# solislemuslab/BayesianNetworkRegression.jl

Measured on AMD Instinct MI355X. Metric: Gibbs iterations/sec (all chains), higher is better.
Workload: dtype f64; 1 GPU; synthetic n=500 V=100 (q=5050) R=7, 8 chains total, 8 per GPU; chains_total=8, chains_per_gpu=8, seed=20240501

## Files before the change

### bayesiannetworkregression.jl_amd/csrc/bnr_kernels.h

```cpp
#pragma once
#include "bnr_device.h"

#define BNR_RMAX 32
#define BNR_NB 32
#define BNR_GT 64


#define BNR_GLOBAL_PTR(member) d.member = (decltype(d.member))(__attribute__((address_space(1))) void *)(unsigned long long)(d.member)
__device__ __forceinline__ bnr_dev bnr_globalized(const bnr_dev *src)
{
    bnr_dev d = *src;
    BNR_GLOBAL_PTR(X); BNR_GLOBAL_PTR(X8); BNR_GLOBAL_PTR(XM); BNR_GLOBAL_PTR(Sdig); BNR_GLOBAL_PTR(y); BNR_GLOBAL_PTR(ek); BNR_GLOBAL_PTR(el); BNR_GLOBAL_PTR(trace); BNR_GLOBAL_PTR(plan);
    BNR_GLOBAL_PTR(pbase); BNR_GLOBAL_PTR(Wbuf); BNR_GLOBAL_PTR(sz); BNR_GLOBAL_PTR(PW); BNR_GLOBAL_PTR(PA); BNR_GLOBAL_PTR(PG);
    BNR_GLOBAL_PTR(Gpart); BNR_GLOBAL_PTR(E); BNR_GLOBAL_PTR(gmap); BNR_GLOBAL_PTR(a3); BNR_GLOBAL_PTR(xw); BNR_GLOBAL_PTR(a4);
    BNR_GLOBAL_PTR(res); BNR_GLOBAL_PTR(xg); BNR_GLOBAL_PTR(bw); BNR_GLOBAL_PTR(wv); BNR_GLOBAL_PTR(scal); BNR_GLOBAL_PTR(Minv);
    BNR_GLOBAL_PTR(Psum); BNR_GLOBAL_PTR(counters); BNR_GLOBAL_PTR(dbg); BNR_GLOBAL_PTR(stamp); BNR_GLOBAL_PTR(gprog); BNR_GLOBAL_PTR(gmapc); BNR_GLOBAL_PTR(dfctl);
    return d;
}
struct bnr_one {
    bnr_dev d;
    static constexpr bool whole = true, lone = true;
    __device__ __forceinline__ const bnr_dev &get() const { return d; }
    __device__ __forceinline__ const bnr_dev &get_x() const { return d; }
    __device__ __forceinline__ const bnr_dev &at(int) const { return d; }
// ... 423 lines not shown
            int f = wave_chol(sA, R, lane);
            if (f && lane == 0) { atomicAdd((unsigned long long *)&cd.counters[3], 1ull); atomicAdd((unsigned long long *)&cd.counters[6], 1ull); }
            const double lgm = (lane < R) ? 2.0 * log(sA[lane + R * lane]) : 0.0;
            double ldm = 0.0;
            for (int i = 0; i < R; ++i) ldm += bnr_readlane_u(lgm, i);
            wave_tri_inverse(sA, sT, R, lane);
            for (int idx = lane; idx < RR; idx += 64) {
                int a = idx % R, b = idx / R, k0 = a > b ? a : b;
                double sacc = 0.0;
                for (int k = k0; k < R; ++k) sacc += sT[k + R * a] * sT[k + R * b];
                cd.Minv[idx] = sacc;
            }
            if (lane == 0) cd.Minv[RR] = ldm;
        }
    }
    if (cap) atomicAdd((unsigned long long *)&cd.counters[2], 1ull);
}

template <class SRC>
__global__ __launch_bounds__(256) void k_xpass(const SRC chain_src, int s, int which, int nchains)
{
    extern __shared__ double sh[];
    const int gid = blockIdx.x;
    const int gx = gid & 7, gr = gid >> 3;
    const int bid = (gr / nchains) * 8 + gx;
    const bnr_dev &cd = chain_src.at(gr % nchains);
    if (bid >= cd.nblk_x) return;
    BNR_TL_IN(cd, TL_XPASS, bid == 0);
    double *sW = sh, *sZ = sh + cd.chunk_x, *sG = sh + 2 * cd.chunk_x;
    const bnr_plan_entry P = cd.plan[cd.pbase[0] + s];
    const double *row = cd.trace + (size_t)P.row * cd.rowlen;
    const double *prev = cd.trace + (size_t)P.prev * cd.rowlen;
    const int R = cd.R;
    const int e0 = bid * cd.chunk_x;
    const int ne = min(cd.chunk_x, cd.q - e0);
    const double *grow = (which & 8) ? prev : row;
    for (int t = threadIdx.x; t < cd.chunk_x; t += blockDim.x) {
        double w = 0.0, zz = 0.0, g = 0.0;
        int e = e0 + t;
        if (t < ne) {
            if (which & 1) { w = edge_W(row + cd.o_u, prev + cd.o_lam, R, cd.el[e], cd.ek[e]); cd.Wbuf[e] = w; }
            if (which & 2) { zz = sqrt(prev[cd.o_S + e]) * bnr_normal(cd.seed, P.it, SITE_G_Z1, (uint32_t)e, 0); cd.sz[e] = zz; }
            if (which & 4) g = grow[cd.o_gamma + e];
        }
        sW[t] = w; sZ[t] = zz; sG[t] = g;
    }
    __syncthreads();
    const size_t ld = cd.n_pad;
    for (int i = threadIdx.x; i < cd.n_pad; i += blockDim.x) {
        double aw = 0.0, aa = 0.0, ag = 0.0;
#define BNR_XPASS_BODY(XP)                                                                                          \
        if ((which & 7) == 3) {                                                                                     \
            _Pragma("unroll 4") for (int t = 0; t < ne; ++t) { double x = (double)(XP)[(size_t)t * ld]; aw = fma(x, sW[t], aw); aa = fma(x, sZ[t], aa); } \
        } else {                                                                                                    \
            for (int t = 0; t < ne; ++t) {                                                                          \
                double x = (double)(XP)[(size_t)t * ld];                                                            \
                aw = fma(x, sW[t], aw); aa = fma(x, sZ[t], aa); ag = fma(x, sG[t], ag);                             \
            }                                                                                                       \
        }
        if (cd.X8) { const unsigned char *xp = cd.X8 + (size_t)e0 * ld + i; BNR_XPASS_BODY(xp) }
        else { const double *xp = cd.X + (size_t)e0 * ld + i; BNR_XPASS_BODY(xp) }
        if (which & 1) cd.PW[(size_t)bid * ld + i] = aw;
        if (which & 2) cd.PA[(size_t)bid * ld + i] = aa;
        if (which & 4) cd.PG[(size_t)bid * ld + i] = ag;
    }
    BNR_TL_OUT(cd, TL_XPASS);
}

__global__ __launch_bounds__(256) void k_xpass_group(const bnr_many chain_src, int s, int nchains)
{
    extern __shared__ double sh[];
    const int wg = blockIdx.x;
    const bnr_dev &c0 = chain_src.at(0);
    const int rs = (c0.n_pad + 255) / 256, bid = wg / rs, slice = wg % rs, tid = threadIdx.x;
    const int chunk = c0.chunk_x, e0 = bid * chunk, ne = min(chunk, c0.q - e0), R = c0.R;
    const size_t ld = c0.n_pad;
    double *sW = sh, *sZ = sh + 8 * chunk;
    __shared__ double *s_pw[8], *s_pa[8];
    const int i = slice * 256 + tid;
    const bool live = i < c0.n_pad;
    const int ic = live ? i : 0;
    for (int cb = 0; cb < nchains; cb += 8) {
        const int nc = min(8, nchains - cb);
        __syncthreads();
        for (int it = tid; it < nc * chunk; it += 256) {
            const int c = it / chunk, t = it - c * chunk;
            const bnr_dev &cd = chain_src.at(cb + c);
            const bnr_plan_entry P = cd.plan[cd.pbase[0] + s];
            const double *row = cd.trace + (size_t)P.row * cd.rowlen, *prev = cd.trace + (size_t)P.prev * cd.rowlen;
            double w = 0.0, zz = 0.0;
            if (t < ne) {
                const int e = e0 + t;
                w = edge_W(row + cd.o_u, prev + cd.o_lam, R, cd.el[e], cd.ek[e]);
                zz = sqrt(prev[cd.o_S + e]) * bnr_normal(cd.seed, P.it, SITE_G_Z1, (uint32_t)e, 0);
                if (slice == 0) { cd.Wbuf[e] = w; cd.sz[e] = zz; }
            }
            sW[c * chunk + t] = w; sZ[c * chunk + t] = zz;
        }
        if (tid < nc) { const bnr_dev &cd = chain_src.at(cb + tid); s_pw[tid] = cd.PW; s_pa[tid] = cd.PA; }
        __syncthreads();
        double aw[8], aa[8];
#pragma unroll
        for (int c = 0; c < 8; ++c) { aw[c] = 0.0; aa[c] = 0.0; }
#define BNR_XG_BODY(XP)                                                                                   \
        for (int t0 = 0; t0 < ne; t0 += 16) {                                                             \
            double xv[16];                                                                                \
            _Pragma("unroll") for (int u = 0; u < 16; ++u) xv[u] = (double)(XP)[(size_t)(t0 + u < ne ? t0 + u : ne - 1) * ld]; \
            _Pragma("unroll") for (int u = 0; u < 16; ++u) {                                              \
                if (t0 + u < ne) {                                                                        \
                    _Pragma("unroll") for (int c = 0; c < 8; ++c)                                         \
                        if (c < nc) { aw[c] = fma(xv[u], sW[c * chunk + t0 + u], aw[c]); aa[c] = fma(xv[u], sZ[c * chunk + t0 + u], aa[c]); } \
                }                                                                                         \
            }                                                                                             \
        }
        if (c0.X8) { const unsigned char *xp = c0.X8 + (size_t)e0 * ld + ic; BNR_XG_BODY(xp) }
        else { const double *xp = c0.X + (size_t)e0 * ld + ic; BNR_XG_BODY(xp) }
#pragma unroll
        for (int c = 0; c < 8; ++c)
            if (c < nc && live) { s_pw[c][(size_t)bid * ld + i] = aw[c]; s_pa[c][(size_t)bid * ld + i] = aa[c]; }
    }
}

typedef int bnr_i4 __attribute__((ext_vector_type(4)));
typedef int bnr_i2 __attribute__((ext_vector_type(2)));
__device__ __forceinline__ __amdgpu_buffer_rsrc_t bnr_rsrc(const void *base)
{
    return __builtin_amdgcn_make_buffer_rsrc((void *)base, 0, 0x7FFFFFFF, 0x00020000);
}
__device__ __forceinline__ bnr_d2 bnr_bufload_d2(__amdgpu_buffer_rsrc_t r, unsigned voff, int soff)
{
    return __builtin_bit_cast(bnr_d2, __builtin_amdgcn_raw_buffer_load_b128(r, (int)voff, soff, 0));
}
__device__ __forceinline__ double bnr_bufload_f64(__amdgpu_buffer_rsrc_t r, unsigned voff, int soff)
{
    return __builtin_bit_cast(double, __builtin_amdgcn_raw_buffer_load_b64(r, (int)voff, soff, 0));
}
__device__ __forceinline__ void bnr_gram_count(const bnr_dev &cd, int tj)
{
    (void)cd; (void)tj;
}
#define BNR_GRAM_KB 16
#define BNR_GRAM_LOOKAHEAD 2
#define BNR_GRAM_PREFETCH_COLS 64
static_assert((BNR_GRAM_LOOKAHEAD + 1) * BNR_GRAM_KB <= BNR_GRAM_PREFETCH_COLS, "zero padding behind X and S must cover the Gram loops' prefetch distance (a half batch + two whole ones)");
__host__ __device__ inline long long bnr_gram_span_bytes(int n_pad, int kchunk, int kg)
{
    return ((long long)(kchunk / kg) + BNR_GRAM_PREFETCH_COLS + 16) * (long long)n_pad * 8;
}

__device__ __forceinline__ void bnr_gstore(double *p, double v) { *p = v; }
struct bnr_gram_geom { const double *X; int n_pad, q_pad, ksplit, q, ntile; };
__device__ __forceinline__ bnr_gram_geom bnr_geom_of(const bnr_dev &cd) { return bnr_gram_geom{cd.X, cd.n_pad, cd.q_pad, cd.ksplit, cd.q, cd.ntile}; }
template <int KG>
__device__ __forceinline__ void bnr_gram16_task(const bnr_gram_geom &cd, const double *Sp, double *Gpart, int t, int ti, int tj, int ks, double *sred)
{
    const int wave = threadIdx.x >> 6, lane = threadIdx.x & 63;
    const int kg = wave >> 2, wi = (wave >> 1) & 1, wj = wave & 1;
    const int kchunk = cd.q_pad / cd.ksplit;
    const int ksub = kchunk / KG;
    const int eb = ks * kchunk + kg * ksub;
    const int nfull = ksub / BNR_GRAM_KB;
    const bool half = (ksub % BNR_GRAM_KB) != 0;
    const size_t ld = cd.n_pad;
    const int li = lane & 15, lk = lane >> 4;
    const int tg = threadIdx.x & 255, c = tg >> 5, rp = tg & 31;
    const unsigned offI = 8u * ((unsigned)(ti * BNR_GT + 2 * rp) + (unsigned)c * (unsigned)ld), offJ = 8u * ((unsigned)(tj * BNR_GT + 2 * rp) + (unsigned)c * (unsigned)ld);
    const unsigned off8 = 8u * 8u * (unsigned)ld, offS = 8u * (unsigned)c;
    const double *xb = bnr_sgpr_global(cd.X + (size_t)eb * ld);
    const double *sb = bnr_sgpr_global(Sp + eb);
    const int PANEL = BNR_GRAM_KB * BNR_GT;
    double *stg = sred + (size_t)kg * (4 * PANEL);
    const int woff = c * BNR_GT + ((2 * rp) ^ ((c & 1) << 4));
    const int sw = (lk & 1) << 4;
    const int ra0 = (wj * 32 + li) ^ sw, ra1 = (wj * 32 + 16 + li) ^ sw, rb0 = (wi * 32 + li) ^ sw, rb1 = (wi * 32 + 16 + li) ^ sw;
    bnr_d4 c00 = {0, 0, 0, 0}, c01 = {0, 0, 0, 0}, c10 = {0, 0, 0, 0}, c11 = {0, 0, 0, 0};
    bnr_d2 ri0, ri1, rj0, rj1;
    double sv0, sv1;
    const __amdgpu_buffer_rsrc_t rX = bnr_rsrc(xb), rS = bnr_rsrc(sb);
    const int bstep = BNR_GRAM_KB * (int)ld * 8;
#define BNR_GRAM_LOAD(BIDX)                                                                               \
    do {                                                                                                  \
        const int so_ = (BIDX) * bstep;                                                                   \
        sv0 = bnr_bufload_f64(rS, offS, (BIDX) * (BNR_GRAM_KB * 8)); sv1 = bnr_bufload_f64(rS, offS + 64u, (BIDX) * (BNR_GRAM_KB * 8)); \
        ri0 = bnr_bufload_d2(rX, offI, so_); ri1 = bnr_bufload_d2(rX, offI + off8, so_);                  \
        rj0 = bnr_bufload_d2(rX, offJ, so_); rj1 = bnr_bufload_d2(rX, offJ + off8, so_);                  \
    } while (0)
#define BNR_GRAM_STORE(BUF)                                                                               \
    do {                                                                                                  \
        double *nx_ = stg + (size_t)(BUF) * (2 * PANEL);                                                  \
        *(bnr_d2 *)(nx_ + woff) = ri0 * sv0;                                                          \
        *(bnr_d2 *)(nx_ + 8 * BNR_GT + woff) = ri1 * sv1;                                             \
        *(bnr_d2 *)(nx_ + PANEL + woff) = rj0;                                                            \
        *(bnr_d2 *)(nx_ + PANEL + 8 * BNR_GT + woff) = rj1;                                               \
    } while (0)
#define BNR_GRAM_COMPUTE(BUF, K2A, K2B, DIAG)                                                                 \
    do {                                                                                                  \
        const double *bufI = stg + (size_t)(BUF) * (2 * PANEL), *bufJ = bufI + PANEL;                     \
        _Pragma("unroll") for (int k2 = (K2A); k2 < (K2B); ++k2) {                                        \
            const int kk = (4 * k2 + lk) * BNR_GT;                                                        \
            double a0 = bufJ[kk + ra0], a1 = bufJ[kk + ra1];                                              \
            double b0 = bufI[kk + rb0], b1 = bufI[kk + rb1];                                              \
            c00 = __builtin_amdgcn_mfma_f64_16x16x4f64(a0, b0, c00, 0, 0, 0);                             \
            c01 = __builtin_amdgcn_mfma_f64_16x16x4f64(a0, b1, c01, 0, 0, 0);                             \
            if (!(DIAG)) c10 = __builtin_amdgcn_mfma_f64_16x16x4f64(a1, b0, c10, 0, 0, 0);                \
            c11 = __builtin_amdgcn_mfma_f64_16x16x4f64(a1, b1, c11, 0, 0, 0);                             \
        }                                                                                                 \
    } while (0)
    BNR_GRAM_LOAD(0);
    BNR_GRAM_STORE(0);
    BNR_GRAM_LOAD(1);
    __syncthreads();
    if (ti == tj && wi == 0 && wj == 1) {
        int b = 0;
        for (; b + 1 < nfull; b += 2) {
            BNR_GRAM_STORE(1); BNR_GRAM_LOAD(b + 2); __syncthreads();
            BNR_GRAM_STORE(0); BNR_GRAM_LOAD(b + 3); __syncthreads();
        }
        if (b < nfull) { BNR_GRAM_STORE(1); BNR_GRAM_LOAD(b + 2); __syncthreads(); }
        if (half) __syncthreads();
    } else if (ti == tj && wi == wj) {
#define BNR_GRAM_BATCH_L(B, PAR, DIAG)                                                                    \
        do {                                                                                              \
            BNR_GRAM_COMPUTE(PAR, 0, 2, DIAG);                                                            \
            BNR_GRAM_STORE((PAR) ^ 1);                                                                    \
            BNR_GRAM_LOAD((B) + 2);                                                                       \
            BNR_GRAM_COMPUTE(PAR, 2, 4, DIAG);                                                            \
            __syncthreads();                                                                              \
        } while (0)
        int b = 0;
        for (; b + 1 < nfull; b += 2) { BNR_GRAM_BATCH_L(b, 0, true); BNR_GRAM_BATCH_L(b + 1, 1, true); }
        if (b < nfull) BNR_GRAM_BATCH_L(b, 0, true);
        if (half) { if (nfull & 1) BNR_GRAM_COMPUTE(1, 0, 2, true); else BNR_GRAM_COMPUTE(0, 0, 2, true); __syncthreads(); }
    } else {
    int b = 0;
    for (; b + 1 < nfull; b += 2) { BNR_GRAM_BATCH_L(b, 0, false); BNR_GRAM_BATCH_L(b + 1, 1, false); }
    if (b < nfull) BNR_GRAM_BATCH_L(b, 0, false);
    if (half) { if (nfull & 1) BNR_GRAM_COMPUTE(1, 0, 2, false); else BNR_GRAM_COMPUTE(0, 0, 2, false); __syncthreads(); }
    }
    double *mine = sred + (size_t)kg * (BNR_GT * BNR_GT);
    const int jb = wj * 32 + (lane >> 4), ib = wi * 32 + (lane & 15);
#pragma unroll
    for (int r = 0; r < 4; ++r) {
        mine[(jb + 4 * r) * BNR_GT + ib] = c00[r];
        mine[(jb + 4 * r) * BNR_GT + ib + 16] = c01[r];
        mine[(jb + 16 + 4 * r) * BNR_GT + ib] = c10[r];
        mine[(jb + 16 + 4 * r) * BNR_GT + ib + 16] = c11[r];
    }
    __syncthreads();
    double *out = Gpart + ((size_t)ks * (cd.ntile * (cd.ntile + 1) / 2) + t) * (BNR_GT * BNR_GT);
#pragma unroll
    for (int idx = threadIdx.x; idx < BNR_GT * BNR_GT; idx += KG * 256) {
        if (KG == 4) bnr_gstore(out + idx, (sred[idx] + sred[BNR_GT * BNR_GT + idx]) + (sred[2 * BNR_GT * BNR_GT + idx] + sred[3 * BNR_GT * BNR_GT + idx]));
        else bnr_gstore(out + idx, sred[idx] + sred[BNR_GT * BNR_GT + idx]);
    }
}
template <class SRC, int KG>
__global__ __launch_bounds__(KG * 256, 4 / KG) void k_gram(const SRC chain_src, int s, int nchains)
{
    const int gid = blockIdx.x, gx = gid & 7, gr = gid >> 3;
    const int gchain = gr % nchains, gslot = (gr / nchains) * 8 + gx;
    const bnr_dev &cd = chain_src.at(gchain);
    __shared__ double sred[KG * BNR_GT * BNR_GT];
    const bnr_plan_entry P = cd.plan[cd.pbase[0] + s];
    const double *Sp = cd.trace + (size_t)P.prev * cd.rowlen + cd.o_S;
    if (gslot >= cd.ksplit * (cd.ntile * (cd.ntile + 1) / 2)) return;
    const int task = cd.gmap[gslot];
    int t = task & 0xFFFF, ti = 0;
    const int ks = task >> 16;
    while ((ti + 1) * (ti + 2) / 2 <= t) ++ti;
    int tj = t - ti * (ti + 1) / 2;
    BNR_TL_IN(cd, TL_GRAM, gslot == 0);
    bnr_gram16_task<KG>(bnr_geom_of(cd), Sp, cd.Gpart, t, ti, tj, ks, sred);
    bnr_gram_count(cd, tj);
    BNR_TL_OUT(cd, TL_GRAM);
}

__device__ __forceinline__ void bnr_gram8_task(const bnr_gram_geom &cd, const double *Sp, double *Gpart, int t, int ti, int tj, int ks, double *sred, unsigned long long *clk = nullptr)
{
    constexpr int KG = 2, KB = 8;
    const int tid = threadIdx.x;
    const int wave = tid >> 6, lane = tid & 63;
    const int kg = wave >> 2, wi = (wave >> 1) & 1, wj = wave & 1;
    const int kchunk = cd.q_pad / cd.ksplit;
    const int ksub = kchunk / KG;
    const int eb = ks * kchunk + kg * ksub;
    const int nbatch = ksub / KB;
    const size_t ld = cd.n_pad;
    const int li = lane & 15, lk = lane >> 4;
    const int tg = tid & 255, c = tg >> 5, rp = tg & 31;
    const unsigned offI = 8u * ((unsigned)(ti * BNR_GT + 2 * rp) + (unsigned)c * (unsigned)ld), offJ = 8u * ((unsigned)(tj * BNR_GT + 2 * rp) + (unsigned)c * (unsigned)ld);
    const unsigned offS = 8u * (unsigned)c;
    const double *xb = bnr_sgpr_global(cd.X + (size_t)eb * ld);
    const double *sb = bnr_sgpr_global(Sp + eb);
    constexpr int PANEL = KB * BNR_GT;
    typedef __attribute__((address_space(3))) double lds_f64;
    typedef __attribute__((address_space(3))) bnr_d2 lds_d2;
    const int sw = (lk & 1) << 4;
    lds_f64 *const stg = (lds_f64 *)sred + kg * (4 * PANEL);
    lds_f64 *pw = stg + c * BNR_GT + ((2 * rp) ^ ((c & 1) << 4));
    lds_f64 *pa0 = stg + PANEL + lk * BNR_GT + ((wj * 32 + li) ^ sw), *pa1 = stg + PANEL + lk * BNR_GT + ((wj * 32 + 16 + li) ^ sw);
    lds_f64 *pb0 = stg + lk * BNR_GT + ((wi * 32 + li) ^ sw), *pb1 = stg + lk * BNR_GT + ((wi * 32 + 16 + li) ^ sw);
    asm volatile("" : "+v"(pw), "+v"(pa0), "+v"(pa1), "+v"(pb0), "+v"(pb1));
    bnr_d4 c00 = {0, 0, 0, 0}, c01 = {0, 0, 0, 0}, c10 = {0, 0, 0, 0}, c11 = {0, 0, 0, 0};
    bnr_d2 ri0, rj0, ri1, rj1;
    double sv0, sv1;
    const __amdgpu_buffer_rsrc_t rX = bnr_rsrc(xb), rS = bnr_rsrc(sb);
    const int bstep = KB * (int)ld * 8;
#define BNR_G8_LOAD(SET, BIDX)                                                               \
    do {                                                                                      \
        sv##SET = bnr_bufload_f64(rS, offS, (BIDX) * (KB * 8));                               \
        ri##SET = bnr_bufload_d2(rX, offI, (BIDX) * bstep);                                   \
        rj##SET = bnr_bufload_d2(rX, offJ, (BIDX) * bstep);                                   \
    } while (0)
#define BNR_G8_STORE(SET, BUF)                                                                \
    do {                                                                                      \
        *(lds_d2 *)(pw + (BUF) * (2 * PANEL)) = ri##SET * sv##SET;                            \
        *(lds_d2 *)(pw + (BUF) * (2 * PANEL) + PANEL) = rj##SET;                              \
    } while (0)
#define BNR_G8_READ(BUF)                                                                      \
    constexpr int o0_ = (BUF) * (2 * PANEL), o1_ = o0_ + 4 * BNR_GT;                          \
    const double a00 = pa0[o0_], a01 = pa0[o1_], a10 = pa1[o0_], a11 = pa1[o1_];              \
    const double b00 = pb0[o0_], b01 = pb0[o1_], b10 = pb1[o0_], b11 = pb1[o1_]
#define BNR_G8_MFMA(K2, DIAG)                                                                 \
    do {                                                                                      \
        c00 = __builtin_amdgcn_mfma_f64_16x16x4f64(a0##K2, b0##K2, c00, 0, 0, 0);             \
        c01 = __builtin_amdgcn_mfma_f64_16x16x4f64(a0##K2, b1##K2, c01, 0, 0, 0);             \
        if (!(DIAG)) c10 = __builtin_amdgcn_mfma_f64_16x16x4f64(a1##K2, b0##K2, c10, 0, 0, 0); \
        c11 = __builtin_amdgcn_mfma_f64_16x16x4f64(a1##K2, b1##K2, c11, 0, 0, 0);             \
    } while (0)
    BNR_G8_LOAD(0, 0);
    BNR_G8_STORE(0, 0);
    BNR_G8_LOAD(1, 1);
    __syncthreads();
#ifdef BNR_STAMPS
    if (clk && tid == 0) { clk[0] = __builtin_amdgcn_s_memtime(); clk[1] = __builtin_amdgcn_s_memrealtime(); }
#endif
#define BNR_G8_BATCH_L(B, PAR, NPAR, DIAG)                                                    \
    do {                                                                                      \
        BNR_G8_LOAD(PAR, (B) + 2);                                                            \
        __builtin_amdgcn_sched_barrier(0);                                                    \
        BNR_G8_READ(PAR);                                                                     \
        BNR_G8_MFMA(0, DIAG);                                                                 \
        __builtin_amdgcn_sched_barrier(0);                                                    \
        BNR_G8_STORE(NPAR, NPAR);                                                             \
        __builtin_amdgcn_sched_barrier(0);                                                    \
        BNR_G8_MFMA(1, DIAG);                                                                 \
        __builtin_amdgcn_sched_barrier(0);                                                    \
        __syncthreads();                                                                      \
    } while (0)
#define BNR_G8_BATCH_DEAD(B, PAR, NPAR)                                                       \
    do {                                                                                      \
        BNR_G8_LOAD(PAR, (B) + 2);                                                            \
        __builtin_amdgcn_sched_barrier(0);                                                    \
        BNR_G8_STORE(NPAR, NPAR);                                                             \
        __syncthreads();                                                                      \
    } while (0)
    if (ti == tj && wi == 0 && wj == 1) {
        int b = 0;
        for (; b + 1 < nbatch; b += 2) { BNR_G8_BATCH_DEAD(b, 0, 1); BNR_G8_BATCH_DEAD(b + 1, 1, 0); }
        if (b < nbatch) BNR_G8_BATCH_DEAD(b, 0, 1);
    } else if (ti == tj && wi == wj) {
        int b = 0;
        for (; b + 1 < nbatch; b += 2) { BNR_G8_BATCH_L(b, 0, 1, true); BNR_G8_BATCH_L(b + 1, 1, 0, true); }
        if (b < nbatch) BNR_G8_BATCH_L(b, 0, 1, true);
    } else {
        int b = 0;
        for (; b + 1 < nbatch; b += 2) { BNR_G8_BATCH_L(b, 0, 1, false); BNR_G8_BATCH_L(b + 1, 1, 0, false); }
        if (b < nbatch) BNR_G8_BATCH_L(b, 0, 1, false);
    }
#ifdef BNR_STAMPS
    if (clk && tid == 0) { clk[2] = __builtin_amdgcn_s_memtime(); clk[3] = __builtin_amdgcn_s_memrealtime(); }
#endif
    int tid_e = tid;
    asm volatile("" : "+v"(tid_e));
    const int jb = ((tid_e >> 6) & 1) * 32 + ((tid_e & 63) >> 4), ib = ((tid_e >> 7) & 1) * 32 + (tid_e & 15);
    if (kg == 1) {
#pragma unroll
        for (int r = 0; r < 4; ++r) {
            sred[(jb + 4 * r) * BNR_GT + ib] = c00[r];
            sred[(jb + 4 * r) * BNR_GT + ib + 16] = c01[r];
            sred[(jb + 16 + 4 * r) * BNR_GT + ib] = c10[r];
            sred[(jb + 16 + 4 * r) * BNR_GT + ib + 16] = c11[r];
        }
    }
    __syncthreads();
    if (kg == 0) {
        double *out = Gpart + ((size_t)ks * (cd.ntile * (cd.ntile + 1) / 2) + t) * (BNR_GT * BNR_GT);
#pragma unroll
        for (int r = 0; r < 4; ++r) {
            bnr_gstore(out + (jb + 4 * r) * BNR_GT + ib, c00[r] + sred[(jb + 4 * r) * BNR_GT + ib]);
            bnr_gstore(out + (jb + 4 * r) * BNR_GT + ib + 16, c01[r] + sred[(jb + 4 * r) * BNR_GT + ib + 16]);
            bnr_gstore(out + (jb + 16 + 4 * r) * BNR_GT + ib, c10[r] + sred[(jb + 16 + 4 * r) * BNR_GT + ib]);
            bnr_gstore(out + (jb + 16 + 4 * r) * BNR_GT + ib + 16, c11[r] + sred[(jb + 16 + 4 * r) * BNR_GT + ib + 16]);
        }
    }
}
template <class SRC>
__global__ __launch_bounds__(512, 6) void k_gram8(const SRC chain_src, int s, int nchains)
{
    const int gid = blockIdx.x, gx = gid & 7, gr = gid >> 3;
    const int gchain = gr % nchains, gslot = (gr / nchains) * 8 + gx;
    const bnr_dev &cd = chain_src.at(gchain);
    __shared__ double sred[BNR_GT * BNR_GT];
    const bnr_plan_entry P = cd.plan[cd.pbase[0] + s];
    const double *Sp = cd.trace + (size_t)P.prev * cd.rowlen + cd.o_S;
    if (gslot >= cd.ksplit * (cd.ntile * (cd.ntile + 1) / 2)) return;
    const int task = cd.gmap[gslot];
    int t = task & 0xFFFF, ti = 0;
    const int ks = task >> 16;
    while ((ti + 1) * (ti + 2) / 2 <= t) ++ti;
    int tj = t - ti * (ti + 1) / 2;
    BNR_TL_IN(cd, TL_GRAM, gslot == 0);
#ifdef BNR_STAMPS
    bnr_gram8_task(bnr_geom_of(cd), Sp, cd.Gpart, t, ti, tj, ks, sred, gslot < 256 ? cd.dbg + 2048 + 4 * gslot : nullptr);
#else
    bnr_gram8_task(bnr_geom_of(cd), Sp, cd.Gpart, t, ti, tj, ks, sred);
#endif
    bnr_gram_count(cd, tj);
    BNR_TL_OUT(cd, TL_GRAM);
}

__global__ void k_x_mask(const unsigned char *X8, int n, int n_pad, int q, int kchunk, int kcp, int kslab, unsigned char *XM, int *not_binary)
{
    const size_t idx = (size_t)blockIdx.x * blockDim.x + threadIdx.x;
    const int ng = kslab / 16;
    if (idx >= (size_t)n_pad * ng) return;
    const int i = (int)(idx / ng), g = (int)(idx % ng);
    const int ks = (16 * g) / kcp, kk0 = (16 * g) % kcp;
    bnr_i4 out = {0, 0, 0, 0};
    bool bad = false;
    for (int b = 0; b < 16; ++b) {
        const int kk = kk0 + b, k = ks * kchunk + kk;
        unsigned v = 0;
        if (i < n && kk < kchunk && k < q) v = X8[(size_t)i + (size_t)n_pad * k];
        if (v > 1u) bad = true;
        if (v) out[b >> 2] |= 0xFF << (8 * (b & 3));
    }
    *(bnr_i4 *)(XM + (size_t)i * kslab + 16 * (size_t)g) = out;
    if (bad) *not_binary = 1;
}
#define BNR_I8_RS 144
#define BNR_I8_TB (64 * BNR_I8_RS)
__host__ __device__ inline size_t bnr_i8_lds_bytes(int L, int kcp) { return (size_t)4 * BNR_I8_TB + (size_t)L * kcp; }
template <int BASE>
__device__ __forceinline__ int bnr_row_bcast(int v, const int l)
{
    switch (BASE + l) {
    case 0: return __builtin_amdgcn_update_dpp(0, v, 0x150, 0xF, 0xF, false);
    case 1: return __builtin_amdgcn_update_dpp(0, v, 0x151, 0xF, 0xF, false);
    case 2: return __builtin_amdgcn_update_dpp(0, v, 0x152, 0xF, 0xF, false);
    case 3: return __builtin_amdgcn_update_dpp(0, v, 0x153, 0xF, 0xF, false);
    case 4: return __builtin_amdgcn_update_dpp(0, v, 0x154, 0xF, 0xF, false);
    case 5: return __builtin_amdgcn_update_dpp(0, v, 0x155, 0xF, 0xF, false);
    case 6: return __builtin_amdgcn_update_dpp(0, v, 0x156, 0xF, 0xF, false);
    case 7: return __builtin_amdgcn_update_dpp(0, v, 0x157, 0xF, 0xF, false);
    case 8: return __builtin_amdgcn_update_dpp(0, v, 0x158, 0xF, 0xF, false);
    case 9: return __builtin_amdgcn_update_dpp(0, v, 0x159, 0xF, 0xF, false);
    case 10: return __builtin_amdgcn_update_dpp(0, v, 0x15A, 0xF, 0xF, false);
    case 11: return __builtin_amdgcn_update_dpp(0, v, 0x15B, 0xF, 0xF, false);
    case 12: return __builtin_amdgcn_update_dpp(0, v, 0x15C, 0xF, 0xF, false);
    case 13: return __builtin_amdgcn_update_dpp(0, v, 0x15D, 0xF, 0xF, false);
    case 14: return __builtin_amdgcn_update_dpp(0, v, 0x15E, 0xF, 0xF, false);
    default: return __builtin_amdgcn_update_dpp(0, v, 0x15F, 0xF, 0xF, false);
    }
}
template <class SRC, int L>
__global__ __launch_bounds__(256, 2) void k_gram_i8(const SRC chain_src, int s, int nchains)
{
    const int gid = blockIdx.x, gx = gid & 7, gr = gid >> 3;
    const int gchain = gr % nchains, gslot = (gr / nchains) * 8 + gx;
    const bnr_dev &cd = chain_src.at(gchain);
    const int ntl = cd.ntile * (cd.ntile + 1) / 2;
    if (gslot >= cd.ksplit * ntl) return;
    const int task = cd.gmap[gslot];
    int t = task & 0xFFFF, ti = 0;
    const int ks = task >> 16;
    while ((ti + 1) * (ti + 2) / 2 <= t) ++ti;
    const int tj = t - ti * (ti + 1) / 2;
    extern __shared__ bnr_i4 smem_i8[];
    unsigned char *sX = (unsigned char *)smem_i8;
    bnr_i4 *sDig = (bnr_i4 *)(sX + 4 * BNR_I8_TB);
    const int tid = threadIdx.x, wave = tid >> 6, lane = tid & 63, ln = lane & 15, lq = lane >> 4;
    const int ng = cd.kcp / 16;
    for (int idx = tid; idx < L * ng; idx += 256) {
        const int l = idx / ng, g = idx % ng;
        sDig[idx] = *(const bnr_i4 *)(cd.Sdig + (size_t)l * cd.kslab + (size_t)ks * cd.kcp + 16 * g);
    }
    const int srow = tid >> 3, scol = tid & 7;
    const unsigned char *gI = cd.XM + (size_t)(ti * BNR_GT + srow) * cd.kslab + (size_t)ks * cd.kcp + 16 * scol;
    const unsigned char *gJ = cd.XM + (size_t)(tj * BNR_GT + srow) * cd.kslab + (size_t)ks * cd.kcp + 16 * scol;
    const size_t r32 = (size_t)32 * cd.kslab;
    const int soff = srow * BNR_I8_RS + 16 * scol;
    bnr_i4 r0 = {0, 0, 0, 0}, r1 = r0, r2 = r0, r3 = r0;
    const int nbatch = cd.kcp / 128, nb = nbatch + ((cd.kcp % 128) ? 1 : 0);
    auto load = [&](int b) {
        const int o = 128 * b;
        if (b < nbatch || scol < 4) { r0 = *(const bnr_i4 *)(gI + o); r1 = *(const bnr_i4 *)(gI + r32 + o); r2 = *(const bnr_i4 *)(gJ + o); r3 = *(const bnr_i4 *)(gJ + r32 + o); }
    };
    auto store = [&](int buf) {
        unsigned char *d = sX + buf * 2 * BNR_I8_TB + soff;
        *(bnr_i4 *)d = r0; *(bnr_i4 *)(d + 32 * BNR_I8_RS) = r1; *(bnr_i4 *)(d + BNR_I8_TB) = r2; *(bnr_i4 *)(d + BNR_I8_TB + 32 * BNR_I8_RS) = r3;
    };
    bnr_i4 acc[L][4];
#pragma unroll
    for (int l = 0; l < L; ++l)
#pragma unroll
        for (int a = 0; a < 4; ++a) acc[l][a] = bnr_i4{0, 0, 0, 0};
    load(0); store(0);
    if (nb > 1) load(1);
    __syncthreads();
    const int fa = ln * BNR_I8_RS + 16 * lq + BNR_I8_TB, fb = (wave * 16 + ln) * BNR_I8_RS + 16 * lq;
    for (int b = 0; b < nb; ++b) {
        const unsigned char *xb = sX + (b & 1) * 2 * BNR_I8_TB;
        const int nk = (b < nbatch) ? 2 : 1;
        bnr_i4 dgall;
        {
            const int pl = ln & 7, pk = ln >> 3, lcl = pl < L ? pl : L - 1;
            int gi = (2 * b + pk) * 4 + lq;
            gi = gi < ng ? gi : ng - 1;
            dgall = sDig[lcl * ng + gi];
        }
#pragma unroll
        for (int kk = 0; kk < 2; ++kk) {
            if (kk >= nk) break;
            const bnr_i4 a0 = *(const bnr_i4 *)(xb + fa + 64 * kk), a1 = *(const bnr_i4 *)(xb + fa + 16 * BNR_I8_RS + 64 * kk);
            const bnr_i4 a2 = *(const bnr_i4 *)(xb + fa + 32 * BNR_I8_RS + 64 * kk), a3 = *(const bnr_i4 *)(xb + fa + 48 * BNR_I8_RS + 64 * kk);
            const bnr_i4 b0 = *(const bnr_i4 *)(xb + fb + 64 * kk);
#pragma unroll
// ... 691 lines not shown
        const double *pAA = E + (size_t)pa + orow + ld * (size_t)pa + ocol, *pBA = E + (size_t)pb + orow + ld * (size_t)pa + ocol;
        const double *pBB = E + (size_t)pb + orow + ld * (size_t)pb + ocol;
        const double *pOA = E + (size_t)(R * BNR_NB) + orow + ld * (size_t)pa + ocol, *pOB = E + (size_t)(R * BNR_NB) + orow + ld * (size_t)pb + ocol;
#pragma unroll
        for (int r = 0; r < 4; ++r) {
            const size_t o = ld * (size_t)(4 * r);
            cAA[r] = pAA[o]; cBA[r] = pBA[o]; cBB[r] = pBB[o]; cOA[r] = pOA[o]; cOB[r] = pOB[o];
        }
        if (P > 0) {
#pragma unroll
            for (int qq = 0; qq < 2; ++qq) {
                const size_t kc = ld * (size_t)((a - 2 + qq) * BNR_NB);
                double ca[8], cb[8], ra[8], rb[8], ro[8];
#pragma unroll
                for (int ks = 0; ks < 8; ++ks) {
                    const size_t o = kc + (size_t)ln + ld * (size_t)(4 * ks + lq);
                    ca[ks] = E[(size_t)(pa + mt * 16) + o]; cb[ks] = E[(size_t)(pb + mt * 16) + o];
                    ra[ks] = E[(size_t)(pa + nt * 16) + o]; rb[ks] = E[(size_t)(pb + nt * 16) + o];
                    ro[ks] = E[(size_t)(R * BNR_NB + nt * 16) + o];
                }
#pragma unroll
                for (int ks = 0; ks < 8; ++ks) {
                    cAA = __builtin_amdgcn_mfma_f64_16x16x4f64(-ca[ks], ra[ks], cAA, 0, 0, 0);
                    cBA = __builtin_amdgcn_mfma_f64_16x16x4f64(-ca[ks], rb[ks], cBA, 0, 0, 0);
                    cBB = __builtin_amdgcn_mfma_f64_16x16x4f64(-cb[ks], rb[ks], cBB, 0, 0, 0);
                    cOA = __builtin_amdgcn_mfma_f64_16x16x4f64(-ca[ks], ro[ks], cOA, 0, 0, 0);
                    cOB = __builtin_amdgcn_mfma_f64_16x16x4f64(-cb[ks], ro[ks], cOB, 0, 0, 0);
                }
            }
        }
#pragma unroll
        for (int r = 0; r < 4; ++r) {
            const int o = (nt * 16 + ln) + BNR_LP * (mt * 16 + lq + 4 * r);
            sh.sDaa[o] = cAA[r]; sh.sDba[o] = cBA[r]; sh.sDbb[o] = cBB[r]; sh.sOa[o] = cOA[r]; sh.sOb[o] = cOB[r];
        }
    }
    __syncthreads();
    int bad = 0;
    double a1[16], a2[16];
    const int rr = lane & 31;
    double *sBw = wave == 0 ? sh.sOa : sh.sDba;
    if (wave < 2) {
        bnr_panel_load16(a1, sh.sDaa, sBw, lane, 0);
        bad = bnr_sweep16<0>(a1, lane);
#pragma unroll
        for (int c = 0; c < 16; ++c) sh.sL1[wave][c * BNR_L1S + lane] = a1[c];
    }
    __syncthreads();
    if (wave < 2) bnr_mid_tile(sh.sDaa, wave * 16, sh.sL1[0], wave * 16, ln, lq);
    else {
        double *sX = wave == 2 ? sh.sOa : sh.sDba;
        bnr_mid_tile(sX, 0, sh.sL1[wave - 2], 32, ln, lq);
        bnr_mid_tile(sX, 16, sh.sL1[wave - 2], 48, ln, lq);
    }
    __syncthreads();
    if (wave < 2) {
        bnr_panel_load16(a2, sh.sDaa, sBw, lane, 16);
        bad |= bnr_sweep16<16>(a2, lane);
        if (lane >= 32) {
#pragma unroll
            for (int c = 0; c < 16; ++c) { sBw[rr + BNR_LP * c] = a1[c]; sBw[rr + BNR_LP * (16 + c)] = a2[c]; }
        }
    }
    __syncthreads();
    {
        const int mt = wave >> 1, nt = wave & 1;
        bnr_lds_tile_update(sh.sDbb, sh.sDba, sh.sDba, mt, nt, ln, lq);
        bnr_lds_tile_update(sh.sOb, sh.sDba, sh.sOa, mt, nt, ln, lq);
    }
    __syncthreads();
    if (wave == 0) {
        bnr_panel_load16(a1, sh.sDbb, sh.sOb, lane, 0);
        bad |= bnr_sweep16<0>(a1, lane);
#pragma unroll
        for (int c = 0; c < 16; ++c) sh.sL1[0][c * BNR_L1S + lane] = a1[c];
    }
    __syncthreads();
    bnr_mid_tile(wave < 2 ? sh.sDbb : sh.sOb, (wave & 1) * 16, sh.sL1[0], 16 * wave, ln, lq);
    __syncthreads();
    if (wave == 0) {
        bnr_panel_load16(a2, sh.sDbb, sh.sOb, lane, 16);
        bad |= bnr_sweep16<16>(a2, lane);
        if (lane >= 32) {
#pragma unroll
            for (int c = 0; c < 16; ++c) { sh.sOb[rr + BNR_LP * c] = a1[c]; sh.sOb[rr + BNR_LP * (16 + c)] = a2[c]; }
        }
    }
    __syncthreads();
    if (bad && tid == 0) bnr_flag_gfail(cd);
    {
        const int r = tid & 31, c0 = tid >> 5;
#pragma unroll
        for (int mm = 0; mm < 4; ++mm) {
            const int c = c0 + 8 * mm;
            if (!only_b) E[(size_t)(R * BNR_NB + r) + ld * (size_t)(pa + c)] = sh.sOa[r + BNR_LP * c];
            E[(size_t)(R * BNR_NB + r) + ld * (size_t)(pb + c)] = sh.sOb[r + BNR_LP * c];
        }
    }
}

template <class SRC>
__global__ __launch_bounds__(256) void k_rhs(const SRC chain_src, int s)
{
    const bnr_dev &cd = chain_src.get();
    __shared__ double sw[4][64], sa[4][64];
    const bnr_plan_entry P = cd.plan[cd.pbase[0] + s];
    const double *prev = cd.trace + (size_t)P.prev * cd.rowlen;
    const double tau = cd.scal[SC_TAU], mu = prev[ROW_MU];
    const int n = cd.n;
    const size_t ld = cd.n_pad;
    const int il = threadIdx.x & 63, g = threadIdx.x >> 6, i = blockIdx.x * 64 + il;
    BNR_TL_IN(cd, TL_RHS, blockIdx.x == 0);
    double xw = 0.0, xs = 0.0;
    const int nb = cd.nblk_x;
    int b = g;
    for (; b + 60 < nb; b += 64) {
        double w[16], a[16];
#pragma unroll
        for (int u = 0; u < 16; ++u) { w[u] = cd.PW[(size_t)(b + 4 * u) * ld + i]; a[u] = cd.PA[(size_t)(b + 4 * u) * ld + i]; }
#pragma unroll
        for (int u = 0; u < 16; ++u) { xw += w[u]; xs += a[u]; }
    }
    for (; b + 12 < nb; b += 16) {
        double w[4], a[4];
#pragma unroll
        for (int u = 0; u < 4; ++u) { w[u] = cd.PW[(size_t)(b + 4 * u) * ld + i]; a[u] = cd.PA[(size_t)(b + 4 * u) * ld + i]; }
#pragma unroll
        for (int u = 0; u < 4; ++u) { xw += w[u]; xs += a[u]; }
    }
    for (; b < nb; b += 4) { xw += cd.PW[(size_t)b * ld + i]; xs += cd.PA[(size_t)b * ld + i]; }
    sw[g][il] = xw; sa[g][il] = xs;
    __syncthreads();
    if (g == 0) {
        xw = (sw[0][il] + sw[1][il]) + (sw[2][il] + sw[3][il]);
        xs = (sa[0][il] + sa[1][il]) + (sa[2][il] + sa[3][il]);
        double z2 = (i < n) ? bnr_normal(cd.seed, P.it, SITE_G_Z2, (uint32_t)i, 0) : 0.0;
        double bb = (i < n) ? ((cd.y[i] - xw - mu) / tau - (xs + z2)) : 0.0;
        cd.xw[i] = xw; cd.a3[i] = xs;
        cd.bw[i] = bb;
    }
    BNR_TL_OUT(cd, TL_RHS);
}
template <class SRC>
__global__ __launch_bounds__(256) void k_solve_w(const SRC chain_src)
{
    BNR_CRITICAL_PATH();
    const bnr_dev &cd = chain_src.get();
    const int wave = threadIdx.x >> 6, lane = threadIdx.x & 63, np = cd.n_pad;
    const int c = blockIdx.x * 4 + wave;
    BNR_TL_IN(cd, TL_SOLVE_W, blockIdx.x == 0);
    const size_t ld = bnr_ldE(np);
    const double *col = cd.E + (size_t)np + ld * (size_t)c;
    const int rend = (c / BNR_NB + 1) * BNR_NB;
    double acc = 0.0;
    for (int r = lane; r < rend; r += 64) acc = fma(col[r], cd.bw[r], acc);
    acc = wave_sum(acc);
    if (lane == 0) cd.wv[c] = acc;
    if (blockIdx.x == 0 && threadIdx.x == 0 && cd.counters[9]) {
        cd.counters[9] = 0;
        atomicAdd((unsigned long long *)&cd.counters[3], 1ull); atomicAdd((unsigned long long *)&cd.counters[7], 1ull);
    }
    BNR_TL_OUT(cd, TL_SOLVE_W);
}
template <class SRC>
__global__ __launch_bounds__(1024) void k_solve_a4(const SRC chain_src)
{
    BNR_CRITICAL_PATH();
    const bnr_dev &cd = chain_src.get();
    extern __shared__ double shs[];
    double *swv = shs, *spart = shs + cd.n_pad;
    const int np = cd.n_pad, tid = threadIdx.x;
    const size_t ld = bnr_ldE(np);
    const int rb = blockIdx.x, rl = tid & 31, cg = tid >> 5;
    const int cstart = rb * BNR_NB;
    BNR_TL_IN(cd, TL_SOLVE_A4, rb == 0);
    for (int c = cstart + tid; c < np; c += 1024) swv[c] = cd.wv[c];
    __syncthreads();
    const double *yrow = cd.E + (size_t)(np + rb * BNR_NB + rl);
    double acc0 = 0.0, acc1 = 0.0;
    int c = cstart + cg;
    for (; c + 32 < np; c += 64) { acc0 = fma(yrow[ld * (size_t)c], swv[c], acc0); acc1 = fma(yrow[ld * (size_t)(c + 32)], swv[c + 32], acc1); }
    if (c < np) acc0 = fma(yrow[ld * (size_t)c], swv[c], acc0);
    spart[cg * 33 + rl] = acc0 + acc1;
    __syncthreads();
    if (tid < 32) {
        double a4 = 0.0;
#pragma unroll
        for (int g = 0; g < 32; ++g) a4 += spart[g * 33 + tid];
        const int r = rb * BNR_NB + tid;
        const double tau = cd.scal[SC_TAU], bb = cd.bw[r];
        cd.a4[r] = a4;
        cd.xg[r] = (r < cd.n) ? (cd.xw[r] + tau * cd.a3[r] + tau * (bb - a4)) : 0.0;
    }
    BNR_TL_OUT(cd, TL_SOLVE_A4);
}

template <class SRC>
__global__ __launch_bounds__(256) void k_backproj(const SRC chain_src, int s, int flags, int nchains, int nslot)
{
    BNR_CRITICAL_PATH();
    const int gid = blockIdx.x, gx = gid & 7, gr = gid >> 3;
    const int bid = (gr / nchains) * 8 + gx;
    const bnr_dev &cd = chain_src.at(gr % nchains);
    if (bid >= cd.nblk_bp) return;
    extern __shared__ double sh[];
    double *sa = sh, *sdot = sh + cd.n_pad;
    const bnr_plan_entry P = cd.plan[cd.pbase[0] + s];
    double *row = cd.trace + (size_t)P.row * cd.rowlen;
    const double *prev = cd.trace + (size_t)P.prev * cd.rowlen;
    const int R = cd.R, tid = threadIdx.x, wave = tid >> 6, lane = tid & 63;
    const int e0 = bid * cd.chunk_bp, ne = min(cd.chunk_bp, cd.q - e0);
    const size_t ld = cd.n_pad;
    const double tau2 = row[ROW_TAU2], tau = sqrt(tau2);
#ifdef BNR_STAMPS
#define BNR_BSTAMP(slot) do { if (tid == 0 && bid == 7) cd.dbg[320 + (slot)] = __builtin_amdgcn_s_memtime(); } while (0)
#else
#define BNR_BSTAMP(slot) do { } while (0)
#endif
    BNR_BSTAMP(0);
#ifdef BNR_STAMPS
    if (tid == 0 && bid < 1800) cd.dbg[400 + 2 * bid] = __builtin_amdgcn_s_memrealtime();
#endif
    BNR_TL_IN(cd, (flags & 3) ? TL_BACKPROJ : TL_PSUM, bid == 0);
    __shared__ double sdr[BNR_RMAX * 33];
    if (flags & 4) {
        const double *un0 = row + cd.o_u;
        for (int idx = tid; idx < R * 32; idx += blockDim.x) {
            const int r = idx >> 5, ee = idx & 31;
            double v = 0.0;
            if (ee < ne) { const int l0 = cd.el[e0 + ee], k0 = cd.ek[e0 + ee]; v = un0[r + R * l0] * un0[r + R * k0]; }
            sdr[r * 33 + ee] = v;
        }
    }
    if (flags & 1) {
        for (int i = tid; i < cd.n_pad; i += blockDim.x) sa[i] = cd.a4[i];
        __syncthreads();
        if (flags & 256)
        for (int t = wave; t < ne; t += 16) {
            const int t2 = t + 4, t3 = t + 8, t4 = t + 12;
            const size_t oc = (size_t)(e0 + t) * ld, od = (size_t)(e0 + (t2 < ne ? t2 : t)) * ld, oe = (size_t)(e0 + (t3 < ne ? t3 : t)) * ld, of = (size_t)(e0 + (t4 < ne ? t4 : t)) * ld;
            double acc0 = 0.0, acc1 = 0.0, acc2 = 0.0, acc3 = 0.0;
            if (cd.X8) {
                const unsigned char *xc = cd.X8 + oc, *xd = cd.X8 + od, *xe = cd.X8 + oe, *xf = cd.X8 + of;
#pragma unroll 4
                for (int i = lane; i < cd.n_pad; i += 64) { double av = sa[i]; acc0 = fma((double)xc[i], av, acc0); acc1 = fma((double)xd[i], av, acc1); acc2 = fma((double)xe[i], av, acc2); acc3 = fma((double)xf[i], av, acc3); }
            } else {
                const double *xc = cd.X + oc, *xd = cd.X + od, *xe = cd.X + oe, *xf = cd.X + of;
#pragma unroll 4
                for (int i = lane; i < cd.n_pad; i += 64) { double av = sa[i]; acc0 = fma(xc[i], av, acc0); acc1 = fma(xd[i], av, acc1); acc2 = fma(xe[i], av, acc2); acc3 = fma(xf[i], av, acc3); }
            }
            acc0 = wave_sum(acc0); acc1 = wave_sum(acc1); acc2 = wave_sum(acc2); acc3 = wave_sum(acc3);
            if (lane == 0) { sdot[t] = acc0; if (t2 < ne) sdot[t2] = acc1; if (t3 < ne) sdot[t3] = acc2; if (t4 < ne) sdot[t4] = acc3; }
        }
        else
        for (int t = wave; t < ne; t += 8) {
            const int t2 = t + 4;
            const size_t oc = (size_t)(e0 + t) * ld, od = (size_t)(e0 + (t2 < ne ? t2 : t)) * ld;
            double acc0 = 0.0, acc1 = 0.0;
            if (cd.X8) {
                const unsigned char *xc = cd.X8 + oc, *xd = cd.X8 + od;
#pragma unroll 4
                for (int i = lane; i < cd.n_pad; i += 64) { double av = sa[i]; acc0 = fma((double)xc[i], av, acc0); acc1 = fma((double)xd[i], av, acc1); }
            } else {
                const double *xc = cd.X + oc, *xd = cd.X + od;
#pragma unroll 4
                for (int i = lane; i < cd.n_pad; i += 64) { double av = sa[i]; acc0 = fma(xc[i], av, acc0); acc1 = fma(xd[i], av, acc1); }
            }
            acc0 = wave_sum(acc0); acc1 = wave_sum(acc1);
            if (lane == 0) { sdot[t] = acc0; if (t2 < ne) sdot[t2] = acc1; }
        }
    }
    __syncthreads();
    BNR_BSTAMP(1);
#ifdef BNR_STAMPS
    if (tid == 0 && bid < 1000) cd.dbg[2000 + bid] = __builtin_amdgcn_s_memrealtime();
#endif
    __shared__ double s_val[8][32];
    __shared__ int s_acc[8][32];
    int cap = 0;
    const bool split = nslot >= 4;
    const int nw = split ? nslot >> 1 : 1;
    const int nsk = split ? nw : 2;
    const int dw = split ? 0 : (bid & 3);
    if (split ? wave >= nw : wave != dw) return;
    const int mykind = wave < (nw >> 1) ? 2 : 3, kw = split ? wave - (mykind == 3 ? (nw >> 1) : 0) : 0;
    const int el32 = lane & 31, slot = kw * 2 + (lane >> 5);
    const int e = e0 + el32;
    const bool act = el32 < ne, keeper = wave == dw && lane < 32;
    double gam = 0.0, Snew = 1.0, W = 0.0;
    if (act) {
        W = cd.Wbuf[e];
        if (flags & 1) {
            double Sp = prev[cd.o_S + e];
            gam = tau * (cd.sz[e] + Sp * sdot[el32]) + W;
            if (keeper) row[cd.o_gamma + e] = gam;
        } else gam = row[cd.o_gamma + e];
    }
    if (flags & 2) {
        const double g = gam - W, chi = (g * g) / tau2, psi = prev[ROW_THETA];
        const int kind = act ? bnr_gig_kind(0.5, chi, psi) : 4;
        const bool loop = kind == 2 || kind == 3, mine = split ? kind == mykind : loop;
        bnr_gig_ctx gc;
        gc.kind = 4;
        if (mine || (keeper && act && !loop)) bnr_gig_setup(gc, 0.5, chi, psi);
        bool done = !loop;
        for (uint32_t base = 0; base < BNR_MAX_ATTEMPTS; base += (uint32_t)nsk) {
            double v = 0.0;
            const bool ok = mine && !done && bnr_gig_try(gc, cd.seed, P.it, (uint32_t)e, base + (uint32_t)slot, v);
            if (mine) { s_acc[slot][el32] = ok ? 1 : 0; s_val[slot][el32] = v; }
            if (split) __syncthreads(); else bnr_wsync();
            if (!done) {
#pragma unroll
                for (int a = 7; a >= 0; --a) if (a < nsk && s_acc[a][el32]) { Snew = s_val[a][el32]; done = true; }
            }
            if (split) { if (!__syncthreads_or(done ? 0 : 1)) break; }
            else { bnr_wsync(); if (__ballot(!done) == 0ull) break; }
        }
        if (split ? __syncthreads_or(done ? 0 : 1) != 0 : __ballot(!done) != 0ull) {
            if (mine && !done && slot == 0) s_val[0][el32] = gc.alpha * gc.xm;
            if (split) __syncthreads(); else bnr_wsync();
            if (!done) { cap = 1; Snew = s_val[0][el32]; }
        }
        if (keeper && act && !loop) Snew = bnr_gig_degenerate(gc, cd.seed, chi, psi, P.it, (uint32_t)e, &cap);
        if (keeper && act) row[cd.o_S + e] = Snew;
    } else if (act) Snew = row[cd.o_S + e];
    if (wave != dw) return;
    BNR_BSTAMP(2);
    if (!(flags & 4)) { if (cap && lane < 32) atomicAdd((unsigned long long *)&cd.counters[2], 1ull); return; }
    double *ps = cd.Psum + (size_t)bid * (1 + 3 * R);
    double *st = sh;
    const double *lamp = prev + cd.o_lam;
    const double sd = sqrt(tau2 * Snew), lsd = log(sd) + 0.5 * log(2.0 * BNR_PI);
    if (lane < 32) {
        st[lane] = act ? Snew : 0.0;
        for (int r = 0; r < R; ++r) {
            double dr = sdr[r * 33 + lane];
            double lr = lamp[r];
#pragma unroll
            for (int c = 0; c < 3; ++c) {
                double Wc = W + (bnr_lambda_value(c) - lr) * dr;
                double zz = (gam - Wc) / sd;
                st[(1 + 3 * r + c) * 33 + lane] = act ? (-0.5 * zz * zz - lsd) : 0.0;
            }
        }
    }
// ... 859 lines not shown
```

Before: 22960 iterations/s.

## Rebalance Gram diagonal-tile wave roles and batch loads in triangular solve kernels

On diagonal Gram tiles, the wave-to-subtile role assignment is permuted per K-group so the dead or symmetric subtile work is spread across SIMDs instead of always landing on the same wave. The matching epilogue index math is updated to use the same role. The two triangular-solve kernels (k_solve_w, k_solve_a4) now issue batches of 8 or 16 independent loads before accumulating. In k_solve_a4 the first E-row loads and scalar fetches are hoisted ahead of the shared-memory fill and barrier. This raises memory-level parallelism on latency-bound kernels, at the cost of more registers and clamped redundant loads.

```diff
diff --git a/bayesiannetworkregression.jl_amd/csrc/bnr_kernels.h b/bayesiannetworkregression.jl_amd/csrc/bnr_kernels.h
--- a/bayesiannetworkregression.jl_amd/csrc/bnr_kernels.h
+++ b/bayesiannetworkregression.jl_amd/csrc/bnr_kernels.h
@@ -599,10 +599,17 @@
 struct bnr_gram_geom { const double *X; int n_pad, q_pad, ksplit, q, ntile; };
 __device__ __forceinline__ bnr_gram_geom bnr_geom_of(const bnr_dev &cd) { return bnr_gram_geom{cd.X, cd.n_pad, cd.q_pad, cd.ksplit, cd.q, cd.ntile}; }
 template <int KG>
+__device__ __forceinline__ int bnr_gram_role_mask(int kg, int ti, int tj)
+{
+    static_assert(KG == 2 || KG == 4, "role masks are written for two and four K-groups");
+    const int m = (KG == 2 ? 3 * kg : (0x9C >> (2 * kg)) & 3) ^ (ti & 1);
+    return ti == tj ? m : 0;
+}
+template <int KG>
 __device__ __forceinline__ void bnr_gram16_task(const bnr_gram_geom &cd, const double *Sp, double *Gpart, int t, int ti, int tj, int ks, double *sred)
 {
     const int wave = threadIdx.x >> 6, lane = threadIdx.x & 63;
-    const int kg = wave >> 2, wi = (wave >> 1) & 1, wj = wave & 1;
+    const int kg = wave >> 2, role = (wave & 3) ^ bnr_gram_role_mask<KG>(kg, ti, tj), wi = role >> 1, wj = role & 1;
     const int kchunk = cd.q_pad / cd.ksplit;
     const int ksub = kchunk / KG;
     const int eb = ks * kchunk + kg * ksub;
@@ -727,7 +734,7 @@
     constexpr int KG = 2, KB = 8;
     const int tid = threadIdx.x;
     const int wave = tid >> 6, lane = tid & 63;
-    const int kg = wave >> 2, wi = (wave >> 1) & 1, wj = wave & 1;
+    const int kg = wave >> 2, role = (wave & 3) ^ bnr_gram_role_mask<KG>(kg, ti, tj), wi = role >> 1, wj = role & 1;
     const int kchunk = cd.q_pad / cd.ksplit;
     const int ksub = kchunk / KG;
     const int eb = ks * kchunk + kg * ksub;
@@ -820,7 +827,8 @@
 #endif
     int tid_e = tid;
     asm volatile("" : "+v"(tid_e));
-    const int jb = ((tid_e >> 6) & 1) * 32 + ((tid_e & 63) >> 4), ib = ((tid_e >> 7) & 1) * 32 + (tid_e & 15);
+    const int role_e = ((tid_e >> 6) & 3) ^ bnr_gram_role_mask<KG>(tid_e >> 8, ti, tj);
+    const int jb = (role_e & 1) * 32 + ((tid_e & 63) >> 4), ib = (role_e >> 1) * 32 + (tid_e & 15);
     if (kg == 1) {
 #pragma unroll
         for (int r = 0; r < 4; ++r) {
@@ -1818,8 +1826,15 @@
     const size_t ld = bnr_ldE(np);
     const double *col = cd.E + (size_t)np + ld * (size_t)c;
     const int rend = (c / BNR_NB + 1) * BNR_NB;
+    const double *bw = cd.bw;
     double acc = 0.0;
-    for (int r = lane; r < rend; r += 64) acc = fma(col[r], cd.bw[r], acc);
+    for (int r0 = lane; r0 < rend; r0 += 8 * 64) {
+        double yv[8], bv[8];
+#pragma unroll
+        for (int u = 0; u < 8; ++u) { const int r = min(r0 + 64 * u, rend - 1); yv[u] = col[r]; bv[u] = bw[r]; }
+#pragma unroll
+        for (int u = 0; u < 8; ++u) acc = (r0 + 64 * u < rend) ? fma(yv[u], bv[u], acc) : acc;
+    }
     acc = wave_sum(acc);
     if (lane == 0) cd.wv[c] = acc;
     if (blockIdx.x == 0 && threadIdx.x == 0 && cd.counters[9]) {
@@ -1840,23 +1855,47 @@
     const int rb = blockIdx.x, rl = tid & 31, cg = tid >> 5;
     const int cstart = rb * BNR_NB;
     BNR_TL_IN(cd, TL_SOLVE_A4, rb == 0);
-    for (int c = cstart + tid; c < np; c += 1024) swv[c] = cd.wv[c];
-    __syncthreads();
     const double *yrow = cd.E + (size_t)(np + rb * BNR_NB + rl);
+    const int r = rb * BNR_NB + rl;
+    const double *pscal = cd.scal, *pbw = cd.bw, *pxw = cd.xw, *pa3 = cd.a3;
+    asm volatile("" : "+v"(pscal), "+v"(pbw), "+v"(pxw), "+v"(pa3));
+    double yv[16];
+#define BNR_A4_LOAD(C0) _Pragma("unroll") for (int k = 0; k < 16; ++k) yv[k] = yrow[ld * (size_t)min((C0) + 32 * k, np - 1)]
+    int c = cstart + cg;
+    double tau = 0.0, bb = 0.0, xw = 0.0, a3 = 0.0;
+    if (tid < 32) { tau = pscal[SC_TAU]; bb = pbw[r]; xw = pxw[r]; a3 = pa3[r]; }
+    const double w0 = cd.wv[min(cstart + tid, np - 1)];
+    BNR_A4_LOAD(c);
+    if (cstart + tid < np) swv[cstart + tid] = w0;
+    for (int c4 = cstart + tid + 1024; c4 < np; c4 += 4 * 1024) {
+        double wq[4];
+#pragma unroll
+        for (int u = 0; u < 4; ++u) wq[u] = cd.wv[min(c4 + 1024 * u, np - 1)];
+#pragma unroll
+        for (int u = 0; u < 4; ++u) if (c4 + 1024 * u < np) swv[c4 + 1024 * u] = wq[u];
+    }
+    __syncthreads();
     double acc0 = 0.0, acc1 = 0.0;
-    int c = cstart + cg;
-    for (; c + 32 < np; c += 64) { acc0 = fma(yrow[ld * (size_t)c], swv[c], acc0); acc1 = fma(yrow[ld * (size_t)(c + 32)], swv[c + 32], acc1); }
-    if (c < np) acc0 = fma(yrow[ld * (size_t)c], swv[c], acc0);
+    for (;;) {
+#pragma unroll
+        for (int k = 0; k < 16; k += 2) {
+            const int ca = min(c + 32 * k, np - 1), cb = min(c + 32 * k + 32, np - 1);
+            acc0 = (c + 32 * k < np) ? fma(yv[k], swv[ca], acc0) : acc0;
+            acc1 = (c + 32 * k + 32 < np) ? fma(yv[k + 1], swv[cb], acc1) : acc1;
+        }
+        c += 16 * 32;
+        if (c >= np) break;
+        BNR_A4_LOAD(c);
+    }
+#undef BNR_A4_LOAD
     spart[cg * 33 + rl] = acc0 + acc1;
     __syncthreads();
     if (tid < 32) {
         double a4 = 0.0;
 #pragma unroll
         for (int g = 0; g < 32; ++g) a4 += spart[g * 33 + tid];
-        const int r = rb * BNR_NB + tid;
-        const double tau = cd.scal[SC_TAU], bb = cd.bw[r];
         cd.a4[r] = a4;
-        cd.xg[r] = (r < cd.n) ? (cd.xw[r] + tau * cd.a3[r] + tau * (bb - a4)) : 0.0;
+        cd.xg[r] = (r < cd.n) ? (xw + tau * a3 + tau * (bb - a4)) : 0.0;
     }
     BNR_TL_OUT(cd, TL_SOLVE_A4);
 }
```

Result: no change. 23130 iterations/s, median of 6 (+0.7%).
